# facebookresearch/SlowFast

Measured on AMD Instinct MI355X. Metric: clips/sec (fwd+bwd), SlowFast-8x8-R50 32x224^2 synthetic clips, per-GPU batch 32, higher is better.
Workload: dtype fp16; 1 GPU; SLOWFAST_8x8_R50: forward + cross_entropy loss + backward + sgd step, inputs resident in HBM, per-GPU batch 32; global_batch=32, parallelism=dp1, launch=hip-graph(fwd+bwd) + eager all-reduce/optimizer, optimizer=FlatOptimizer (fused unscale+norm+clip+update, dynamic loss scale on device)

## Files before the change

slowfast_amd/csrc/sf_api.hip:

```cpp
#include "../../include/sfamd.h"
#include "sf_bn.h"
#include "sf_common.h"
#include "sf_igemm.h"
#include "sf_igemm2.h"
#include "sf_wgrad2.h"
#include "sf_pool.h"
#include "sf_dwconv.h"
#include "sf_dwsweep.h"
#include "sf_dwtemporal.h"
#include "sf_tokens.h"
#include "sf_x3d.h"
#include "sf_stem.h"
#include "sf_attn.h"
#include "sf_roi.h"
#include "sf_optim.h"

#include <stdarg.h>
#include <stdio.h>
#include <stdlib.h>
#include <string.h>

static thread_local char g_err[512] = "";

static int fail(const char* fmt, ...) {
    va_list ap;
    va_start(ap, fmt);
    vsnprintf(g_err, sizeof(g_err), fmt, ap);
    va_end(ap);
    return -1;
}
static int check_launch(const char* what) {
    hipError_t e = hipGetLastError();
    if (e != hipSuccess) return fail("%s: launch failed: %s", what, hipGetErrorString(e));
    return 0;
}
#define REQUIRE(cond, ...) \
    do { if (!(cond)) return fail(__VA_ARGS__); } while (0)

static inline int cdiv(int64_t a, int64_t b) { return (int)((a + b - 1) / b); }
static inline int roundup(int a, int b) { return (a + b - 1) / b * b; }

static inline int test_hook(const char* name, int def) { const char* e = getenv(name); return e ? atoi(e) : def; }
#ifdef SF_DIAG
static inline int tune_knob(const char* name, int def) { const char* e = getenv(name); return e ? atoi(e) : def; }
#else
#define tune_knob(name, def) (def)
#endif

extern "C" int sf_abi_version(void) { return SF_ABI_VERSION; }
extern "C" const char* sf_backend(void) {
#ifdef SF_HOSTSIM
    return "hostsim";
#else
    return "gfx950";
#endif
}
extern "C" int sf_act_dtype(void) { return SF_ACT_DTYPE_ID; }
extern "C" const char* sf_last_error(void) { return g_err; }
#ifndef SF_BUILD_ID
#define SF_BUILD_ID "unversioned"
#endif
extern "C" const char* sf_build_id(void) {
    static const char tagged[] = "sfamd-build-id:" SF_BUILD_ID;
    return tagged + 15;
}

static int check_desc(const sf_conv_desc* d) {
    REQUIRE(d != nullptr, "conv: null descriptor");
    REQUIRE(d->N > 0 && d->Ci > 0 && d->Co > 0, "conv: empty tensor");
    REQUIRE(d->Ci % 8 == 0 && d->Co % 8 == 0, "conv: channel counts must be multiples of 8 (Ci=%d Co=%d)", d->Ci, d->Co);
    REQUIRE(d->ldx >= d->Ci && d->ldx % 8 == 0 && d->ldy >= d->Co && d->ldy % 8 == 0, "conv: bad row pitch");
    REQUIRE(d->Cw > 0 && d->Cw <= d->Ci, "conv: Cw must be in (0, Ci]");
    REQUIRE(d->Cow >= 0 && d->Cow <= d->Co, "conv: Cow must be in [0, Co]");
    REQUIRE(d->sT > 0 && d->sH > 0 && d->sW > 0 && d->dT > 0 && d->dH > 0 && d->dW > 0, "conv: stride/dilation");
    int To = (d->Ti + 2 * d->pT - d->dT * (d->kT - 1) - 1) / d->sT + 1;
    int Ho = (d->Hi + 2 * d->pH - d->dH * (d->kH - 1) - 1) / d->sH + 1;
    int Wo = (d->Wi + 2 * d->pW - d->dW * (d->kW - 1) - 1) / d->sW + 1;
    REQUIRE(d->To >= 1 && d->Ho >= 1 && d->Wo >= 1 && d->To <= To && d->Ho <= Ho && d->Wo <= Wo,
            "conv: output dims (%d,%d,%d) exceed the geometry's (%d,%d,%d)", d->To, d->Ho, d->Wo, To, Ho, Wo);
    int64_t Mo = (int64_t)d->N * d->To * d->Ho * d->Wo, Mi = (int64_t)d->N * d->Ti * d->Hi * d->Wi;
    REQUIRE(Mo < (1ll << 31) && Mi < (1ll << 31), "conv: more than 2^31 positions");
    return 0;
}

static void fill_gather_common(GatherSide& g, const sf_conv_desc* d) {
    g.kT = d->kT; g.kH = d->kH; g.kW = d->kW;
    g.strT = d->sT; g.strH = d->sH; g.strW = d->sW;
    g.padT = d->pT; g.padH = d->pH; g.padW = d->pW;
    g.dilT = d->dT; g.dilH = d->dH; g.dilW = d->dW;
    g.fdkW = make_fastdiv(d->kW);
    g.fdkH = make_fastdiv(d->kH);
    g.fdsT = make_fastdiv(d->sT);
    g.fdsH = make_fastdiv(d->sH);
    g.fdsW = make_fastdiv(d->sW);
    g.scale = nullptr; g.shift = nullptr; g.relu = 0;
    g.fdHW = make_fastdiv((uint32_t)d->Hi * (uint32_t)d->Wi);
}
static bool is_pointwise(const sf_conv_desc* d) {
    return d->kH == 1 && d->kW == 1 && d->sT == 1 && d->sH == 1 && d->sW == 1 && d->pH == 0 && d->pW == 0 &&
           d->Ho == d->Hi && d->Wo == d->Wi;
}

static GatherSide gather_fwd(const sf_conv_desc* d, const void* x, const float* sc, const float* sh, int relu) {
    GatherSide g;
    memset(&g, 0, sizeof(g));
    fill_gather_common(g, d);
    g.src = (const f16*)x; g.ld = d->ldx; g.C = d->Ci;
    g.sT = d->Ti; g.sH = d->Hi; g.sW = d->Wi;
    g.mode = 0;
    g.Ktot = d->kT * d->kH * d->kW * d->Ci;
    g.fdC = make_fastdiv(d->Ci);
    g.fdrW = make_fastdiv(d->Wo); g.fdrH = make_fastdiv(d->Ho); g.fdrT = make_fastdiv(d->To);
    g.rowT = d->To;
    g.scale = sc; g.shift = sh; g.relu = relu;
    return g;
}
static GatherSide gather_dgrad(const sf_conv_desc* d, const void* dy) {
    GatherSide g;
    memset(&g, 0, sizeof(g));
    fill_gather_common(g, d);
    g.src = (const f16*)dy; g.ld = d->ldy; g.C = d->Co;
    g.sT = d->To; g.sH = d->Ho; g.sW = d->Wo;
    g.mode = 1;
    g.Ktot = d->kT * d->kH * d->kW * d->Co;
    g.fdC = make_fastdiv(d->Co);
    g.fdrW = make_fastdiv(d->Wi); g.fdrH = make_fastdiv(d->Hi); g.fdrT = make_fastdiv(d->Ti);
    g.rowT = d->Ti;
    return g;
}

static bool igemm_glds_ok(const IgemmParams& p, bool pw) {
    static const bool off = tune_knob("SF_IGEMM_GLDS", 1) == 0;
    if (off || !pw || p.g.scale) return false;
    if (p.g.Ktot != p.g.C || p.g.Ktot % 32 != 0 || p.g.ld % 8 != 0 || p.ldw % 8 != 0) return false;
    if (p.g.padT != 0) return false;
    if (((uintptr_t)p.g.src | (uintptr_t)p.wmat) & 15) return false;
    if (p.bh > 0 && ((p.sa_b | p.sa_h | p.sw_b | p.sw_h) & 7)) return false;
    return true;
}

template <int BN, int WM, int WN>
static void launch_igemm(const IgemmParams& p, bool pw, hipStream_t s, int nbatch = 1) {
    int mt = cdiv(p.M, 128);
    dim3 grid((unsigned)(mt * p.ntiles_n), (unsigned)nbatch);
    static const bool occ4 = tune_knob("SF_IGEMM_OCC4", 1) != 0;
    if (p.f32.out) {
        if (igemm_glds_ok(p, pw)) hipLaunchKernelGGL((sf_igemm_kernel<BN, WM, WN, true, true, BN == 128, true>), grid, dim3(SF_THREADS), 0, s, p);
        else hipLaunchKernelGGL((sf_igemm_kernel<BN, WM, WN, true, false, BN == 128, true>), grid, dim3(SF_THREADS), 0, s, p);
        return;
    }
    if (igemm_glds_ok(p, pw)) {
        hipLaunchKernelGGL((sf_igemm_kernel<BN, WM, WN, true, true, BN == 128>), grid, dim3(SF_THREADS), 0, s, p);
        return;
    }
    constexpr bool kCap = BN == 128;
    const bool cap = kCap && occ4;
    if (pw) {
        if (cap) hipLaunchKernelGGL((sf_igemm_kernel<BN, WM, WN, true, false, kCap>), grid, dim3(SF_THREADS), 0, s, p);
        else hipLaunchKernelGGL((sf_igemm_kernel<BN, WM, WN, true, false, false>), grid, dim3(SF_THREADS), 0, s, p);
    } else {
        if (cap) hipLaunchKernelGGL((sf_igemm_kernel<BN, WM, WN, false, false, kCap>), grid, dim3(SF_THREADS), 0, s, p);
        else hipLaunchKernelGGL((sf_igemm_kernel<BN, WM, WN, false, false, false>), grid, dim3(SF_THREADS), 0, s, p);
    }
}

template <int BN, int BK>
static void launch_igemm2(Igemm2Params& q, hipStream_t s) {
    q.ntiles_n = cdiv(q.Nout, BN);
    const dim3 grid((unsigned)(cdiv(q.M, 256) * q.ntiles_n));
    if constexpr (BN >= 64) {
        if (q.f32.out) { hipLaunchKernelGGL((sf_igemm2_kernel<256, BN, 4, 2, BK, 3, true>), grid, dim3(512), 0, s, q); return; }
    }
    hipLaunchKernelGGL((sf_igemm2_kernel<256, BN, 4, 2, BK, 3>), grid, dim3(512), 0, s, q);
}
static void launch_igemm2_auto(Igemm2Params& q, hipStream_t s) {
    const char* e;
    const int tiles = cdiv(q.M, 256) * cdiv(q.Nout, q.Nout > 64 ? 128 : 64);
    const int force_bk = tune_knob("SF_IGEMM2_BK", 0);
    const bool bk64 = q.C % 64 == 0 && force_bk != 32 && (force_bk == 64 || tiles <= 320);
    static const bool trace = test_hook("SF_TRACE", 0) != 0;
    q.ablate = tune_knob("SF_IGEMM2_ABLATE", 0);
    if (trace) fprintf(stderr, "[sfamd] igemm2: M=%d N=%d C=%d taps=%d BK=%d omap=%d\n", q.M, q.Nout, q.C, q.ntaps, bk64 ? 64 : 32, q.omap);
    const int t128 = test_hook("SF_IGEMM2_T128", 1);
    if (t128 && q.linear && q.Nout > 64 && !q.stat_part && !q.bnb_part && (!bk64 || t128 == 2)) {
        q.ntiles_n = cdiv(q.Nout, 128);
        const dim3 grid((unsigned)(cdiv(q.M, 128) * q.ntiles_n));
        if (q.f32.out) hipLaunchKernelGGL((sf_igemm2_kernel<128, 128, 2, 2, 32, 3, true>), grid, dim3(256), 0, s, q);
        else hipLaunchKernelGGL((sf_igemm2_kernel<128, 128, 2, 2, 32, 3>), grid, dim3(256), 0, s, q);
        return;
    }
    if (q.Nout > 64) { if (bk64) launch_igemm2<128, 64>(q, s); else launch_igemm2<128, 32>(q, s); }
    else if (q.Nout > 32) { if (bk64) launch_igemm2<64, 64>(q, s); else launch_igemm2<64, 32>(q, s); }
    else launch_igemm2<32, 32>(q, s);
}
static bool igemm2_operands_ok(const IgemmParams& p, int nbatch) {
    const GatherSide& g = p.g;
    if (nbatch != 1 || g.scale) return false;
    if (p.bh > 1 || (p.bh == 1 && (p.sa_b | p.sa_h | p.sw_b | p.sw_h | p.sy_b | p.sy_h | p.sr_b | p.sr_h))) return false;
    const int taps = g.kT * g.kH * g.kW;
    if (taps > SF_I2_MAXTAPS || g.C % 32 != 0 || g.Ktot != taps * g.C) return false;
    if (g.ld % 8 != 0 || p.ldw % 8 != 0 || p.ldw < g.Ktot) return false;
    if (((uintptr_t)g.src | (uintptr_t)p.wmat) & 15) return false;
    if ((g.kT - 1) * g.dilT > 127 || (g.kH - 1) * g.dilH > 127 || (g.kW - 1) * g.dilW > 127) return false;
    return true;
}
static void igemm2_common(Igemm2Params& q, const IgemmParams& p) {
    const GatherSide& g = p.g;
    memset(&q, 0, sizeof(q));
    q.src = g.src; q.ld = g.ld; q.C = g.C;
    q.sT = g.sT; q.sH = g.sH; q.sW = g.sW;
    q.wmat = p.wmat; q.ldw = p.ldw; q.Nout = p.Nout;
    q.y = p.y; q.ldy = p.ldy; q.bias = p.bias; q.resid = p.resid; q.ldr = p.ldr; q.stat_part = p.stat_part;
    q.act_mode = p.act_mode; q.act_aux = p.act_aux; q.ld_aux = p.ld_aux; q.resid_row0 = p.resid_row0; q.alpha = p.alpha;
    q.resid_bits = p.resid_bits;
    q.bnb_y = p.bnb_y; q.bnb_ld = p.bnb_ld; q.bnb_scale = p.bnb_scale; q.bnb_shift = p.bnb_shift; q.bnb_part = p.bnb_part;
    q.bnb_bits = p.bnb_bits;
    q.f32 = p.f32;
    q.linear = p.linear;
}
static bool try_igemm2(const IgemmParams& p, hipStream_t s, int nbatch = 1) {
    const char* e;
    const bool off = test_hook("SF_IGEMM2", 1) == 0;
    const int mink = test_hook("SF_IGEMM2_MINK", 512);
    const int minrows = test_hook("SF_IGEMM2_MINROWS", 4096);
    const GatherSide& g = p.g;
    if (off || !igemm2_operands_ok(p, nbatch)) return false;
    if (g.Ktot < mink || p.Nout <= 32 || p.M < minrows) return false;
    if (g.mode == 1 && !(g.strT == 1 && g.strH == 1 && g.strW == 1)) return false;
    const int taps = g.kT * g.kH * g.kW;
    Igemm2Params q;
    igemm2_common(q, p);
    q.fdrW = g.fdrW; q.fdrH = g.fdrH; q.fdrT = g.fdrT;
    const int sgn = g.mode == 0 ? 1 : -1;
    if (g.mode == 0) {
        q.mulT = g.strT; q.mulH = g.strH; q.mulW = g.strW;
        q.offT = -g.padT; q.offH = -g.padH; q.offW = -g.padW;
    } else {
        q.mulT = q.mulH = q.mulW = 1;
        q.offT = g.padT; q.offH = g.padH; q.offW = g.padW;
    }
    q.ntaps = taps;
    int t = 0;
    for (int kt = 0; kt < g.kT; ++kt)
        for (int kh = 0; kh < g.kH; ++kh)
            for (int kw = 0; kw < g.kW; ++kw, ++t) {
                const int dt = sgn * kt * g.dilT, dh = sgn * kh * g.dilH, dw = sgn * kw * g.dilW;
                q.dt[t] = (int8_t)dt; q.dh[t] = (int8_t)dh; q.dw[t] = (int8_t)dw;
                q.taps[t].dlin = (dt * g.sH + dh) * g.sW + dw;
                q.taps[t].wcol = t * g.C;
            }
    q.M = p.M;
    launch_igemm2_auto(q, s);
    return true;
}

static bool try_igemm2_strided_dgrad(const IgemmParams& p, hipStream_t s) {
    const char* e;
    const bool off = test_hook("SF_IGEMM2", 1) == 0 || tune_knob("SF_IGEMM2_STRIDED", 1) == 0;
    const int minrows = test_hook("SF_IGEMM2_MINROWS", 4096);
    const GatherSide& g = p.g;
    if (off || g.mode != 1 || (g.strT == 1 && g.strH == 1 && g.strW == 1)) return false;
    if (!igemm2_operands_ok(p, 1) || p.Nout <= 16 || p.M < minrows || p.stat_part || p.act_mode) return false;
    const int Ti = (int)g.fdrT.d, Hi = (int)g.fdrH.d, Wi = (int)g.fdrW.d;
    const int N = p.M / (Ti * Hi * Wi);
    const int str[3] = {g.strT, g.strH, g.strW}, pad[3] = {g.padT, g.padH, g.padW}, dil[3] = {g.dilT, g.dilH, g.dilW};
    const int ker[3] = {g.kT, g.kH, g.kW}, ext[3] = {Ti, Hi, Wi};
    for (int rt = 0; rt < str[0]; ++rt)
        for (int rh = 0; rh < str[1]; ++rh)
            for (int rw = 0; rw < str[2]; ++rw) {
                const int r[3] = {rt, rh, rw};
                int q0[3], cnt[3];
                bool empty = false;
                for (int a = 0; a < 3; ++a) {
                    const int num = pad[a] - r[a];
                    q0[a] = num > 0 ? (num + str[a] - 1) / str[a] : 0;
                    const int top = ext[a] - 1 + pad[a] - r[a];
                    const int q1 = top >= 0 ? top / str[a] : -1;
                    cnt[a] = q1 - q0[a] + 1;
                    if (cnt[a] <= 0) empty = true;
                }
                if (empty) continue;
                Igemm2Params q;
                igemm2_common(q, p);
                q.fdrT = make_fastdiv(cnt[0]); q.fdrH = make_fastdiv(cnt[1]); q.fdrW = make_fastdiv(cnt[2]);
                q.mulT = q.mulH = q.mulW = 1;
                q.offT = q0[0]; q.offH = q0[1]; q.offW = q0[2];
                int nt = 0, tap = 0;
                for (int kt = 0; kt < ker[0]; ++kt)
                    for (int kh = 0; kh < ker[1]; ++kh)
                        for (int kw = 0; kw < ker[2]; ++kw, ++tap) {
                            const int k[3] = {kt, kh, kw};
                            int d[3];
                            bool ok = true;
                            for (int a = 0; a < 3; ++a) {
                                const int v = r[a] - k[a] * dil[a];
                                if (v % str[a] != 0) { ok = false; break; }
                                d[a] = v / str[a];
                            }
                            if (!ok) continue;
                            q.dt[nt] = (int8_t)d[0]; q.dh[nt] = (int8_t)d[1]; q.dw[nt] = (int8_t)d[2];
                            q.taps[nt].dlin = (d[0] * g.sH + d[1]) * g.sW + d[2];
                            q.taps[nt].wcol = tap * g.C;
                            ++nt;
                        }
                q.ntaps = nt;
                q.M = N * cnt[0] * cnt[1] * cnt[2];
                q.omap = 1;
                q.oT = Ti; q.oH = Hi; q.oW = Wi;
                q.omT = str[0]; q.omH = str[1]; q.omW = str[2];
                q.ooT = str[0] * q0[0] + r[0] - pad[0]; q.ooH = str[1] * q0[1] + r[1] - pad[1]; q.ooW = str[2] * q0[2] + r[2] - pad[2];
                launch_igemm2_auto(q, s);
            }
    return true;
}

static int run_igemm(IgemmParams& p, bool pw, hipStream_t s, int* bm_used = nullptr) {
    if (bm_used) *bm_used = 256;
    if (try_igemm2(p, s)) return check_launch("igemm2");
    if (bm_used) *bm_used = 0;
    if (try_igemm2_strided_dgrad(p, s)) return check_launch("igemm2 strided dgrad");
    if (bm_used) *bm_used = 128;
    if (p.Nout > 64) { p.ntiles_n = cdiv(p.Nout, 128); launch_igemm<128, 64, 64>(p, pw, s); }
    else if (p.Nout > 32) { p.ntiles_n = 1; launch_igemm<64, 32, 64>(p, pw, s); }
    else if (p.Nout > 16) { p.ntiles_n = 1; launch_igemm<32, 32, 32>(p, pw, s); }
    else { p.ntiles_n = 1; launch_igemm<16, 32, 16>(p, pw, s); }
    return check_launch("igemm");
}

struct StemPlan {
    bool ok, thin3, small;
    int tiles_w, tiles_h, tiles_t, ntiles, F, PR;
    int wg_blocks, tiles_per_block, Kpad, wgroups;
    size_t ws_bytes;
};
static StemPlan plan_stem(const sf_conv_desc* d) {
    StemPlan s;
    memset(&s, 0, sizeof(s));
    static const bool off = tune_knob("SF_STEM_GENERIC", 0) != 0;
    if (off) return s;
    static const bool thin3_on = tune_knob("SF_STEM_THIN3", 1) != 0;
    const bool stemlike = d->kW == 4 && d->pW == 2;
    const bool thin3 = thin3_on && d->kW == 3 && d->pW == 1 && d->sH == 1 && d->sT == 1;
    if (d->Ci != 8 || d->Cw != 8 || !(stemlike || thin3) || d->sW != 1 || d->dT != 1 || d->dH != 1 || d->dW != 1)
        return s;
    s.thin3 = thin3;
    if (d->Co > 16 || d->Co % 8 != 0 || (d->Cow && d->Cow != d->Co)) return s;
    if (d->kT * d->kH > SF_STEM_MAX_SLICES) return s;
    s.F = (SF_STEM_TT - 1) * d->sT + d->kT;
    s.PR = (SF_STEM_TH - 1) * d->sH + d->kH;
    if ((int64_t)s.F * s.PR * SF_STEM_PC > SF_STEM_CHUNKS) return s;
    s.small = (int64_t)s.F * s.PR * SF_STEM_PC <= SF_STEM_CHUNKS_SMALL;
    s.tiles_w = cdiv(d->Wo, SF_STEM_TW);
    s.tiles_h = cdiv(d->Ho, SF_STEM_TH);
    s.tiles_t = cdiv(d->To, SF_STEM_TT);
    const int64_t nt = (int64_t)d->N * s.tiles_t * s.tiles_h * s.tiles_w;
    if (nt >= (1ll << 30)) return s;
    s.ntiles = (int)nt;
    const int gmax = s.small ? 1024 : 512;
    int g = s.ntiles < gmax ? s.ntiles : gmax;
    s.tiles_per_block = cdiv(s.ntiles, g);
    s.wg_blocks = cdiv(s.ntiles, s.tiles_per_block);
    s.Kpad = roundup(d->kT * d->kH * 32, 128);
    { const int nsl = d->kT * d->kH; s.wgroups = nsl <= 4 ? 8 / nsl : 1; }
    s.ws_bytes = (size_t)s.wg_blocks * s.wgroups * 16 * s.Kpad * 4;
    s.ok = true;
    return s;
}
#define SF_STEM_SLIDE_GROUPS 4
#define SF_STEM_FWD_LAUNCH(sp, q, stream)                                                                                          \
    do {                                                                                                                          \
        static const bool rm_ = tune_knob("SF_STEM_ROWMAJOR", 1) != 0;                           \
        const dim3 g_((sp).ntiles), b_(SF_THREADS);                                                                               \
        const int sg_ = test_hook("SF_STEM_SLIDE", SF_STEM_SLIDE_GROUPS);                                                         \
        if (rm_ && sg_ > 0 && (q).sH == 2 && (q).kH == 7 && !(sp).small && (q).sT == 1 && (q).kT > 1 && (q).kT <= 5 &&            \
            (q).Co <= 8 && !(q).bnb_y) {                                                                                                         \
            StemParams qs_ = (q);                    \
            qs_.seg_groups = sg_ < (sp).tiles_t ? sg_ : (sp).tiles_t;                                                             \
            qs_.tiles_t = cdiv((sp).tiles_t, qs_.seg_groups);                                                                     \
            qs_.fd_tt = make_fastdiv(qs_.tiles_t);                                                                                \
            const dim3 gs_((unsigned)((int64_t)(q).N * qs_.tiles_t * (sp).tiles_h * (sp).tiles_w));                                \
            if (test_hook("SF_TRACE", 0)) fprintf(stderr, "[sfamd] stem_fwd_slide: %u runs of %d groups\n", gs_.x, qs_.seg_groups); \
            hipLaunchKernelGGL((sf_stem_fwd_slide_kernel<2, 7>), gs_, b_, 0, (hipStream_t)(stream), qs_);                         \
        } else if (rm_ && (q).sH == 2 && (q).kH == 7 && !(sp).small)                                                              \
            hipLaunchKernelGGL((sf_stem_fwd_kernel<SF_STEM_CHUNKS, 2, 7>), g_, b_, 0, (hipStream_t)(stream), q);                  \
        else if (rm_ && (q).sH == 1 && (q).kH == 3 && (sp).small)                                                                 \
            hipLaunchKernelGGL((sf_stem_fwd_kernel<SF_STEM_CHUNKS_SMALL, 1, 3>), g_, b_, 0, (hipStream_t)(stream), q);            \
        else if ((sp).small) hipLaunchKernelGGL((sf_stem_fwd_kernel<SF_STEM_CHUNKS_SMALL>), g_, b_, 0, (hipStream_t)(stream), q); \
        else hipLaunchKernelGGL((sf_stem_fwd_kernel<SF_STEM_CHUNKS>), g_, b_, 0, (hipStream_t)(stream), q);                       \
    } while (0)
static StemParams stem_params(const sf_conv_desc* d, const StemPlan& s, const void* x) {
    StemParams p;
    memset(&p, 0, sizeof(p));
    p.x = (const f16*)x; p.ldx = d->ldx;
    p.N = d->N; p.Ti = d->Ti; p.Hi = d->Hi; p.Wi = d->Wi;
    p.To = d->To; p.Ho = d->Ho; p.Wo = d->Wo; p.Co = d->Co;
    p.kT = d->kT; p.kH = d->kH; p.sT = d->sT; p.sH = d->sH; p.pT = d->pT; p.pH = d->pH;
    p.pW = d->pW;
    if (s.thin3) { p.wo0 = 0; p.wos = 24; p.wog = 8; p.kwc = 3; }
    else { p.wo0 = 0; p.wos = 32; p.wog = 8; p.kwc = 4; }
    p.ldy = d->ldy;
    p.tiles_w = s.tiles_w; p.tiles_h = s.tiles_h; p.tiles_t = s.tiles_t; p.ntiles = s.ntiles;
    p.fd_tw = make_fastdiv(s.tiles_w); p.fd_th = make_fastdiv(s.tiles_h); p.fd_tt = make_fastdiv(s.tiles_t);
    p.F = s.F; p.PR = s.PR;
    p.fd_pc = make_fastdiv(SF_STEM_PC); p.fd_prpc = make_fastdiv(s.PR * SF_STEM_PC);
    p.Kpad = s.Kpad; p.tiles_per_block = s.tiles_per_block; p.wgroups = s.wgroups;
    return p;
}

extern "C" int sf_conv_weight_ld(const sf_conv_desc* d, int32_t* ldf, int32_t* ldd) {
    REQUIRE(d && ldf && ldd, "sf_conv_weight_ld: null argument");
    int taps = d->kT * d->kH * d->kW;
    *ldf = roundup(taps * d->Ci, 32);
    *ldd = roundup(taps * d->Co, 32);
    return 0;
}

static PrepParams prep_params(const sf_conv_desc* d, const float* w, void* wf, void* wd) {
    PrepParams p;
    memset(&p, 0, sizeof(p));
    p.w = w; p.Co = d->Co; p.Cow = d->Cow ? d->Cow : d->Co; p.Cw = d->Cw; p.Cp = d->Ci; p.taps = d->kT * d->kH * d->kW;
    int32_t ldf, ldd;
    sf_conv_weight_ld(d, &ldf, &ldd);
    p.wf = (f16*)wf; p.ldf = ldf; p.wd = (f16*)wd; p.ldd = ldd;
    return p;
}

extern "C" int sf_prep_weights(const sf_conv_desc* d, const float* w, void* wf, void* wd, sf_stream_t stream) {
    if (check_desc(d)) return -1;
    REQUIRE(w && wf, "sf_prep_weights: null pointer");
    const PrepParams p = prep_params(d, w, wf, wd);
    int64_t total = (int64_t)p.Co * p.ldf + (wd ? (int64_t)p.Cp * p.ldd : 0);
    int blocks = (int)((total + SF_THREADS - 1) / SF_THREADS);
    if (blocks > 4096) blocks = 4096;
    hipLaunchKernelGGL(sf_prep_weights_kernel, dim3(blocks), dim3(SF_THREADS), 0, (hipStream_t)stream, p);
    return check_launch("prep_weights");
}

static_assert(sizeof(sf_prep_item) == sizeof(PrepParams), "sf_prep_item must mirror PrepParams");
extern "C" int sf_prep_item_fill(const sf_conv_desc* d, const float* w, void* wf, void* wd, sf_prep_item* item) {
    if (check_desc(d)) return -1;
    REQUIRE(w && wf && item, "sf_prep_item_fill: null pointer");
    PrepParams p = prep_params(d, w, wf, wd);
    p.pad = sf_prep_tile_co(p.taps);
    memcpy(item, &p, sizeof(p));
    return 0;
}

extern "C" int64_t sf_prep_item_blocks(const sf_prep_item* item) {
    REQUIRE(item && item->Co > 0 && item->ldf > 0 && item->taps > 0, "sf_prep_item_blocks: bad item");
    REQUIRE(item->pad == sf_prep_tile_co(item->taps), "sf_prep_item_blocks: item was not written by sf_prep_item_fill");
    if (item->pad > 0) return (int64_t)cdiv(item->Co, item->pad) * cdiv(item->Cp, SF_PREP_TILE_CI);
    const int64_t n = (int64_t)item->Co * item->ldf + (item->wd ? (int64_t)item->Cp * item->ldd : 0);
    return cdiv(n, SF_PREP_BLOCK_ELEMS);
}

extern "C" int sf_prep_weights_batch(const sf_prep_item* items, const int32_t* blk_item, const int32_t* blk_off,
                                     int32_t nblocks, sf_stream_t stream) {
    REQUIRE(items && blk_item && blk_off && nblocks > 0, "sf_prep_weights_batch: bad arguments");
    hipLaunchKernelGGL(sf_prep_weights_batch_kernel, dim3(nblocks), dim3(SF_THREADS), 0, (hipStream_t)stream,
                       (const PrepParams*)items, blk_item, blk_off);
    return check_launch("prep_weights_batch");
}

extern "C" int sf_conv_fwd_mtiles(const sf_conv_desc* d) {
    if (!d) return fail("sf_conv_fwd_mtiles: null descriptor");
    return cdiv((int64_t)d->N * d->To * d->Ho * d->Wo, 128);
}

extern "C" int sf_conv_fwd(const sf_conv_desc* d, const void* x, const void* wf, const float* in_scale,
                           const float* in_shift, int in_relu, const float* bias, void* y, float* stat_part,
                           sf_stream_t stream) {
    if (check_desc(d)) return -1;
    REQUIRE(x && wf && y, "sf_conv_fwd: null pointer");
    REQUIRE((in_scale == nullptr) == (in_shift == nullptr), "sf_conv_fwd: in_scale/in_shift must come together");
    REQUIRE(!in_scale || d->Ci <= 512, "sf_conv_fwd: fused input BatchNorm supports Ci <= 512 (got %d)", d->Ci);
    if (!in_scale && !bias) {
        const StemPlan sp = plan_stem(d);
        if (sp.ok && (!stat_part || sp.ntiles <= sf_conv_fwd_mtiles(d))) {
            StemParams q = stem_params(d, sp, x);
            int32_t ldf0, ldd0;
            sf_conv_weight_ld(d, &ldf0, &ldd0);
            q.wmat = (const f16*)wf; q.ldw = ldf0; q.y = (f16*)y;
            q.stat_part = stat_part; q.stat_rows = sf_conv_fwd_mtiles(d);
            const bool trace = test_hook("SF_TRACE", 0) != 0;
            if (trace) fprintf(stderr, "[sfamd] stem_fwd: %d tiles, patch %dx%dx%d chunks\n", sp.ntiles, sp.F, sp.PR, SF_STEM_PC);
            SF_STEM_FWD_LAUNCH(sp, q, stream);
            return check_launch("stem_fwd");
        }
    }
    IgemmParams p;
    memset(&p, 0, sizeof(p));
    p.g = gather_fwd(d, x, in_scale, in_shift, in_relu);
    p.M = d->N * d->To * d->Ho * d->Wo;
    int32_t ldf, ldd;
    sf_conv_weight_ld(d, &ldf, &ldd);
    p.wmat = (const f16*)wf; p.ldw = ldf; p.Nout = d->Co;
    p.ksteps = cdiv(p.g.Ktot, 32);
    p.y = (f16*)y; p.ldy = d->ldy;
    p.bias = bias; p.resid = nullptr; p.ldr = 0;
    p.stat_part = stat_part;
    return run_igemm(p, is_pointwise(d), (hipStream_t)stream);
}

extern "C" int sf_conv_fwd_fused(const sf_conv_desc* d, const void* x, const void* wf, const float* bias,
                                 const void* resid, int32_t ldr, int out_relu, void* y, sf_stream_t stream) {
    if (check_desc(d)) return -1;
    REQUIRE(x && wf && y, "sf_conv_fwd_fused: null pointer");
    REQUIRE(!resid || (ldr >= d->Co && ldr % 8 == 0), "sf_conv_fwd_fused: bad residual pitch");
    if (!resid) {
        const StemPlan sp = plan_stem(d);
        if (sp.ok) {
            StemParams q = stem_params(d, sp, x);
            int32_t ldf0, ldd0;
            sf_conv_weight_ld(d, &ldf0, &ldd0);
            q.wmat = (const f16*)wf; q.ldw = ldf0; q.y = (f16*)y;
            q.bias = bias; q.out_relu = out_relu;
            SF_STEM_FWD_LAUNCH(sp, q, stream);
            return check_launch("stem_fwd_fused");
        }
    }
    IgemmParams p;
    memset(&p, 0, sizeof(p));
    p.g = gather_fwd(d, x, nullptr, nullptr, 0);
    p.M = d->N * d->To * d->Ho * d->Wo;
    int32_t ldf, ldd;
    sf_conv_weight_ld(d, &ldf, &ldd);
    p.wmat = (const f16*)wf; p.ldw = ldf; p.Nout = d->Co;
    p.ksteps = cdiv(p.g.Ktot, 32);
    p.y = (f16*)y; p.ldy = d->ldy;
    p.bias = bias; p.resid = (const f16*)resid; p.ldr = ldr;
    p.act_mode = out_relu ? 3 : 0;
    return run_igemm(p, is_pointwise(d), (hipStream_t)stream);
}

struct BnFuse {
    const float* scale; const float* shift; const void* bits;
    const void* y0; int32_t ld0; float* part0;
};
static int conv_dgrad_impl(const sf_conv_desc* d, const void* dy, const void* wd, const void* resid, int32_t ldr,
                           const void* resid_bits, void* dx, const BnFuse* bn, int32_t* bn_rows, sf_stream_t stream) {
    if (check_desc(d)) return -1;
    REQUIRE(dy && wd && dx, "sf_conv_dgrad: null pointer");
    REQUIRE(!resid || (ldr >= d->Ci && ldr % 8 == 0), "sf_conv_dgrad: bad residual pitch");
    IgemmParams p;
    memset(&p, 0, sizeof(p));
    p.g = gather_dgrad(d, dy);
    p.M = d->N * d->Ti * d->Hi * d->Wi;
    int32_t ldf, ldd;
    sf_conv_weight_ld(d, &ldf, &ldd);
    p.wmat = (const f16*)wd; p.ldw = ldd; p.Nout = d->Ci;
    p.ksteps = cdiv(p.g.Ktot, 32);
    p.y = (f16*)dx; p.ldy = d->ldx;
    p.resid = (const f16*)resid; p.ldr = ldr;
    REQUIRE(!resid_bits || resid, "sf_conv_dgrad: resid_bits without a residual");
    p.resid_bits = (const uint8_t*)resid_bits;
    const bool fuse = bn && d->sT == 1 && d->sH == 1 && d->sW == 1;
    if (!resid && d->Co == 8 && d->To == d->Ti && d->Ho == d->Hi && d->Wo == d->Wi) {
        sf_conv_desc dd = *d;
        dd.Ci = d->Co; dd.Cw = d->Co; dd.Co = d->Ci; dd.Cow = 0;
        dd.pT = d->kT - 1 - d->pT; dd.pH = d->kH - 1 - d->pH; dd.pW = d->kW - 1 - d->pW;
        dd.ldx = d->ldy; dd.ldy = d->ldx;
        const StemPlan sp = plan_stem(&dd);
        if (sp.ok && sp.thin3 && (!fuse || sp.ntiles <= cdiv(p.M, 128))) {
            StemParams q = stem_params(&dd, sp, dy);
            const int S = d->kT * d->kH;
            q.wmat = (const f16*)wd; q.ldw = ldd; q.y = (f16*)dx;
            q.wo0 = ((S - 1) * 3 + 2) * 8; q.wos = -24; q.wog = -8; q.kwc = 3;
            if (fuse) {
                q.bnb_y = (const f16*)bn->y0; q.bnb_ld = bn->ld0; q.bnb_scale = bn->scale; q.bnb_shift = bn->shift;
                q.bnb_bits = (const uint8_t*)bn->bits;
                q.stat_part = bn->part0; q.stat_rows = 0;
            }
            SF_STEM_FWD_LAUNCH(sp, q, stream);
            if (bn_rows) *bn_rows = fuse ? sp.ntiles : 0;
            return check_launch("stem_dgrad");
        }
    }
    if (fuse) {
        p.bnb_y = (const f16*)bn->y0; p.bnb_ld = bn->ld0; p.bnb_part = bn->part0;
        p.bnb_scale = bn->scale; p.bnb_shift = bn->shift; p.bnb_bits = (const uint8_t*)bn->bits;
    }
    int bm = 0;
    const int rc = run_igemm(p, is_pointwise(d), (hipStream_t)stream, &bm);
    if (bn_rows) *bn_rows = (fuse && bm > 0) ? cdiv(p.M, bm) : 0;
    return rc;
}

extern "C" int sf_conv_dgrad(const sf_conv_desc* d, const void* dy, const void* wd, const void* resid, int32_t ldr,
                             const void* resid_bits, void* dx, sf_stream_t stream) {
    return conv_dgrad_impl(d, dy, wd, resid, ldr, resid_bits, dx, nullptr, nullptr, stream);
}

extern "C" int sf_conv_dgrad_bn(const sf_conv_desc* d, const void* dy, const void* wd, const void* resid, int32_t ldr,
                                const void* resid_bits, void* dx, const float* mask_scale, const float* mask_shift,
                                const void* mask_bits, const void* bn_y, int32_t bn_ldy, float* bn_part, int32_t bn_part_rows,
                                int32_t* bn_rows, sf_stream_t stream) {
    REQUIRE(d && bn_y && bn_part && bn_rows, "sf_conv_dgrad_bn: null pointer");
    REQUIRE(mask_bits || (mask_scale && mask_shift), "sf_conv_dgrad_bn: a mask source is needed (mask_bits, or mask_scale + mask_shift)");
    REQUIRE(bn_ldy >= d->Ci && bn_ldy % 8 == 0 && ((uintptr_t)bn_y & 15) == 0, "sf_conv_dgrad_bn: bad bn_y pitch / alignment");
    REQUIRE((int64_t)bn_part_rows * 128 >= (int64_t)d->N * d->Ti * d->Hi * d->Wi,
            "sf_conv_dgrad_bn: the partial table needs ceil(positions / 128) rows of [2][Ci] floats");
    const BnFuse bn = {mask_scale, mask_shift, mask_bits, bn_y, bn_ldy, bn_part};
    return conv_dgrad_impl(d, dy, wd, resid, ldr, resid_bits, dx, &bn, bn_rows, stream);
}

template <int BMW, int WM, int WN, int KS>
static void launch_wgrad(WgradParams& p, dim3 grid3, hipStream_t s) {
    p.tiles_k = grid3.x; p.tiles_c = grid3.y;
    const dim3 grid(grid3.x * grid3.y * grid3.z);
    hipLaunchKernelGGL((sf_wgrad_kernel<BMW, WM, WN, KS>), grid, dim3(SF_THREADS), 0, s, p);
}

struct WgradPlan {
    int BMW, KS, tiles_k, tiles_c, Co_pad, Kpad, nchunks, chunks_per_split, splits;
    size_t ws_bytes;
};
static WgradPlan plan_wgrad(const sf_conv_desc* d) {
    WgradPlan w;
    const int taps = d->kT * d->kH * d->kW;
    const int Ktot = taps * d->Ci;
    const int64_t M = (int64_t)d->N * d->To * d->Ho * d->Wo;
    w.BMW = d->Co >= 128 ? 128 : d->Co >= 64 ? 64 : d->Co >= 32 ? 32 : 16;
    w.KS = w.BMW <= 32 ? 4 : 1;
    w.tiles_k = cdiv(Ktot, 128);
    w.tiles_c = cdiv(d->Co, w.BMW);
    w.Kpad = w.tiles_k * 128;
    w.Co_pad = w.tiles_c * w.BMW;
    w.nchunks = cdiv(M, 32);
    const int64_t slab = (int64_t)w.Co_pad * w.Kpad * 4;
    static const int target = tune_knob("SF_WGRAD_BLOCKS", 1024);
    int splits = cdiv(target, (int64_t)w.tiles_k * w.tiles_c);
    const int64_t cap = (256ll << 20) / slab;
    if (splits > cap) splits = (int)(cap < 1 ? 1 : cap);
    const int nstages = cdiv(w.nchunks, w.KS);
    if (splits > nstages) splits = nstages;
    if (splits < 1) splits = 1;
    w.chunks_per_split = cdiv(nstages, splits) * w.KS;
    w.splits = cdiv(w.nchunks, w.chunks_per_split);
    w.ws_bytes = (size_t)slab * w.splits;
    return w;
}

struct Wgrad2Plan {
    bool ok, thin, dual;
    int BMW, BKW, tiles_k, tiles_c, Co_pad, Kpad, rows_per_split, splits;
    int slabs;
    size_t tab_bytes, ws_bytes;
};
static Wgrad2Plan plan_wgrad2(const sf_conv_desc* d) {
    Wgrad2Plan w;
    memset(&w, 0, sizeof(w));
    const char* e;
    if (test_hook("SF_WGRAD2", 1) == 0) return w;
    const int mink = test_hook("SF_WGRAD2_MINK", 192);
    const int minrows = test_hook("SF_WGRAD2_MINROWS", 4096);
    const int taps = d->kT * d->kH * d->kW;
    const int target = test_hook("SF_WGRAD2_BLOCKS", 512);
    (void)taps;
    const int Ktot = taps * d->Ci;
    const int64_t M = (int64_t)d->N * d->To * d->Ho * d->Wo;
    if (taps > SF_I2_MAXTAPS || M < minrows) return w;
    if ((d->kT - 1) * d->dT > 127 || (d->kH - 1) * d->dH > 127 || (d->kW - 1) * d->dW > 127) return w;
    if (plan_stem(d).ok) return w;
    if (d->Co <= 32) {
        if (test_hook("SF_WGRAD2T", 1) == 0) return w;
        const int minrows_t = test_hook("SF_WGRAD2T_MINROWS", 16384);
        if (M < minrows_t) return w;
        w.thin = true;
        w.BMW = d->Co <= 16 ? 16 : 32;
        w.BKW = Ktot <= 32 ? 32 : 128;
        w.tiles_k = cdiv(Ktot, w.BKW);
        w.tiles_c = 1;
        w.Kpad = w.tiles_k * w.BKW;
        w.Co_pad = w.BMW;
        const int target_t = test_hook("SF_WGRAD2T_BLOCKS", w.BKW == 128 ? 512 : w.BMW == 32 ? 768 : 1024);
        int splits = target_t / w.tiles_k;
        if (splits < 1) splits = 1;
        w.rows_per_split = roundup(cdiv(M, splits), 128);
        w.splits = cdiv(M, w.rows_per_split);
        w.tab_bytes = ((size_t)M * 8 + 255) / 256 * 256 + 1280;
        w.ws_bytes = w.tab_bytes + (size_t)w.Co_pad * w.Kpad * 4 * w.splits;
        w.slabs = w.splits;
        w.ok = true;
        return w;
    }
    if (Ktot < mink) return w;
    w.BMW = d->Co > 64 ? 128 : 64;
    w.tiles_k = cdiv(Ktot, 256);
    w.tiles_c = cdiv(d->Co, w.BMW);
    w.Kpad = w.tiles_k * 256;
    w.Co_pad = w.tiles_c * w.BMW;
    int splits = target / (w.tiles_k * w.tiles_c);
    const int64_t slab = (int64_t)w.Co_pad * w.Kpad * 4;
    const int64_t cap = (256ll << 20) / slab;
    if (splits > cap) splits = (int)(cap < 1 ? 1 : cap);
    if (splits < 1) splits = 1;
    w.dual = false;
    if (splits >= 2 && test_hook("SF_WGRAD2_DUAL", 1) != 0) {
        const int tiles = w.tiles_k * w.tiles_c;
        const int pairs = (target / 2) / tiles;
        const int64_t steps = cdiv(cdiv(M, splits), 32);
        if (pairs >= 1 && 2 * pairs * 10 >= (2 * pairs < splits ? splits : 2 * pairs) * 9 && steps <= test_hook("SF_WGRAD2_DUAL_STEPS", 80)) {
            w.dual = true;
            if (2 * pairs < splits) splits = 2 * pairs;
        }
    }
    w.rows_per_split = roundup(cdiv(M, splits), 32);
    w.splits = cdiv(M, w.rows_per_split);
    if (w.splits < 2) w.dual = false;
    w.slabs = w.dual ? cdiv(w.splits, 2) : w.splits;
    w.tab_bytes = ((size_t)M * 8 + 255) / 256 * 256 + 1280;
    w.ws_bytes = w.tab_bytes + (size_t)slab * w.splits;
    w.ok = true;
    return w;
}

static void launch_rowtab(const sf_conv_desc* d, void* tab, hipStream_t s) {
    RowtabParams t;
    memset(&t, 0, sizeof(t));
    t.tab = (i32x2*)tab;
    t.M = d->N * d->To * d->Ho * d->Wo;
    t.fdW = make_fastdiv(d->Wo); t.fdH = make_fastdiv(d->Ho); t.fdT = make_fastdiv(d->To);
    t.sT = d->Ti; t.sH = d->Hi; t.sW = d->Wi;
    t.strT = d->sT; t.strH = d->sH; t.strW = d->sW; t.padT = d->pT; t.padH = d->pH; t.padW = d->pW;
    t.ntaps = d->kT * d->kH * d->kW;
    int ti = 0;
    for (int kt = 0; kt < d->kT; ++kt)
        for (int kh = 0; kh < d->kH; ++kh)
            for (int kw = 0; kw < d->kW; ++kw, ++ti) {
                t.dt[ti] = (int8_t)(kt * d->dT); t.dh[ti] = (int8_t)(kh * d->dH); t.dw[ti] = (int8_t)(kw * d->dW);
            }
    hipLaunchKernelGGL(sf_wgrad2_rowtab_kernel, dim3(cdiv(t.M, SF_THREADS)), dim3(SF_THREADS), 0, s, t);
}

extern "C" int64_t sf_conv_wgrad_rowtab_bytes(const sf_conv_desc* d) {
    if (check_desc(d)) return -1;
    const Wgrad2Plan w2 = plan_wgrad2(d);
    return w2.ok ? (int64_t)w2.tab_bytes : 0;
}

extern "C" int sf_conv_wgrad_rowtab(const sf_conv_desc* d, void* tab, sf_stream_t stream) {
    if (check_desc(d)) return -1;
    REQUIRE(tab && (uintptr_t)tab % 16 == 0, "sf_conv_wgrad_rowtab: tab must be a 16-byte aligned device pointer");
    REQUIRE(plan_wgrad2(d).ok, "sf_conv_wgrad_rowtab: this geometry does not take the row-table kernel (sf_conv_wgrad_rowtab_bytes == 0)");
    launch_rowtab(d, tab, (hipStream_t)stream);
    return check_launch("wgrad_rowtab");
}

extern "C" int64_t sf_conv_wgrad_workspace(const sf_conv_desc* d) {
    if (check_desc(d)) return -1;
    int64_t generic = (int64_t)plan_wgrad(d).ws_bytes;
    const Wgrad2Plan w2 = plan_wgrad2(d);
    if (w2.ok && (int64_t)w2.ws_bytes > generic) generic = (int64_t)w2.ws_bytes;
    const StemPlan sp = plan_stem(d);
    return sp.ok && (int64_t)sp.ws_bytes > generic ? (int64_t)sp.ws_bytes : generic;
}

extern "C" int sf_conv_wgrad(const sf_conv_desc* d, const void* x, const float* in_scale, const float* in_shift,
                             int in_relu, const void* dy, float* dw, float out_scale, int zero_first,
                             void* workspace, int64_t workspace_bytes, const void* rowtab, sf_stream_t stream) {
    if (check_desc(d)) return -1;
    REQUIRE(x && dy && dw && workspace, "sf_conv_wgrad: null pointer");
    REQUIRE((in_scale == nullptr) == (in_shift == nullptr), "sf_conv_wgrad: in_scale/in_shift must come together");
    REQUIRE(!in_scale || d->Ci <= 512, "sf_conv_wgrad: fused input BatchNorm supports Ci <= 512 (got %d)", d->Ci);
    hipStream_t s = (hipStream_t)stream;
    int splits, Co_pad, Kpad;
    GatherSide gk = gather_fwd(d, x, in_scale, in_shift, in_relu);
    const StemPlan sp = plan_stem(d);
    const Wgrad2Plan w2 = in_scale ? Wgrad2Plan{} : plan_wgrad2(d);
    float* slabs = (float*)workspace;
    if (w2.ok) {
        REQUIRE(workspace_bytes >= (int64_t)w2.ws_bytes, "sf_conv_wgrad: workspace too small (%lld < %lld bytes)",
                (long long)workspace_bytes, (long long)w2.ws_bytes);
        REQUIRE(((uintptr_t)x | (uintptr_t)dy | (uintptr_t)workspace) % 16 == 0, "sf_conv_wgrad: operands must be 16-byte aligned");
        Wgrad2Params q;
        memset(&q, 0, sizeof(q));
        int ti = 0;
        for (int kt = 0; kt < d->kT; ++kt)
            for (int kh = 0; kh < d->kH; ++kh)
                for (int kw = 0; kw < d->kW; ++kw, ++ti) q.dlin[ti] = (kt * d->dT * d->Hi + kh * d->dH) * d->Wi + kw * d->dW;
        if (!rowtab) launch_rowtab(d, workspace, s);
        else REQUIRE((uintptr_t)rowtab % 16 == 0, "sf_conv_wgrad: rowtab must be 16-byte aligned");
        q.x = (const f16*)x; q.ldx = d->ldx; q.C = d->Ci;
        q.dy = (const f16*)dy; q.ldy = d->ldy; q.Co = d->Co;
        q.M = d->N * d->To * d->Ho * d->Wo; q.Ktot = gk.Ktot;
        q.rowtab = (const i32x2*)(rowtab ? rowtab : workspace);
        slabs = (float*)((char*)workspace + w2.tab_bytes);
        q.ws = slabs; q.Co_pad = w2.Co_pad; q.Kpad = w2.Kpad;
        q.tiles_k = w2.tiles_k; q.tiles_c = w2.tiles_c; q.rows_per_split = w2.rows_per_split;
        q.stage_stride = (w2.thin && tune_knob("SF_WGRAD2T_RR", 1) != 0) ? w2.splits : 0;
        const dim3 grid((unsigned)(w2.tiles_k * w2.tiles_c * w2.slabs));
        static const bool trace = test_hook("SF_TRACE", 0) != 0;
        if (trace) fprintf(stderr, "[sfamd] wgrad2: M=%d Co=%d K=%d tiles %dx%d splits %d%s\n", q.M, q.Co, q.Ktot, w2.tiles_c, w2.tiles_k, w2.splits,
                           w2.dual ? " (two per workgroup)" : "");
        if (w2.thin) {
            if (w2.BMW == 16 && w2.BKW == 128) hipLaunchKernelGGL((sf_wgrad2t_kernel<16, 128, 2>), grid, dim3(256), 0, s, q);
            else if (w2.BMW == 32 && w2.BKW == 128) hipLaunchKernelGGL((sf_wgrad2t_kernel<32, 128, 2>), grid, dim3(256), 0, s, q);
            else if (w2.BMW == 16) hipLaunchKernelGGL((sf_wgrad2t_kernel<16, 32, 3>), grid, dim3(256), 0, s, q);
            else hipLaunchKernelGGL((sf_wgrad2t_kernel<32, 32, 3>), grid, dim3(256), 0, s, q);
        } else if (w2.dual) {
            if (w2.BMW == 128) hipLaunchKernelGGL((sf_wgrad2_kernel<128, true>), grid, dim3(1024), 0, s, q);
            else hipLaunchKernelGGL((sf_wgrad2_kernel<64, true>), grid, dim3(1024), 0, s, q);
        } else {
            if (w2.BMW == 128) hipLaunchKernelGGL((sf_wgrad2_kernel<128>), grid, dim3(512), 0, s, q);
            else hipLaunchKernelGGL((sf_wgrad2_kernel<64>), grid, dim3(512), 0, s, q);
        }
        splits = w2.slabs; Co_pad = w2.Co_pad; Kpad = w2.Kpad;
    } else if (sp.ok && !in_scale) {
        REQUIRE(workspace_bytes >= (int64_t)sp.ws_bytes, "sf_conv_wgrad: workspace too small (%lld < %lld bytes)",
                (long long)workspace_bytes, (long long)sp.ws_bytes);
        StemParams q = stem_params(d, sp, x);
        q.dy = (const f16*)dy; q.ws = (float*)workspace;
        const bool trace = test_hook("SF_TRACE", 0) != 0;
        if (trace) fprintf(stderr, "[sfamd] stem_wgrad: %d workgroups x %d tiles\n", sp.wg_blocks, sp.tiles_per_block);
        static const bool stem_plain = tune_knob("SF_STEM_XCD", 1) == 0;
        q.plain_order = stem_plain ? 1 : 0;
        if (d->Co <= 8 && sp.small) hipLaunchKernelGGL((sf_stem_wgrad_kernel<8, SF_STEM_CHUNKS_SMALL>), dim3(sp.wg_blocks), dim3(SF_STEM_WG_THREADS), 0, s, q);
        else if (d->Co <= 8) hipLaunchKernelGGL((sf_stem_wgrad_kernel<8, SF_STEM_CHUNKS>), dim3(sp.wg_blocks), dim3(SF_STEM_WG_THREADS), 0, s, q);
        else if (sp.small) hipLaunchKernelGGL((sf_stem_wgrad_kernel<16, SF_STEM_CHUNKS_SMALL>), dim3(sp.wg_blocks), dim3(SF_STEM_WG_THREADS), 0, s, q);
        else hipLaunchKernelGGL((sf_stem_wgrad_kernel<16, SF_STEM_CHUNKS>), dim3(sp.wg_blocks), dim3(SF_STEM_WG_THREADS), 0, s, q);
        splits = sp.wg_blocks * sp.wgroups; Co_pad = 16; Kpad = sp.Kpad;
    } else {
        const WgradPlan w = plan_wgrad(d);
        REQUIRE(workspace_bytes >= (int64_t)w.ws_bytes, "sf_conv_wgrad: workspace too small (%lld < %lld bytes)",
                (long long)workspace_bytes, (long long)w.ws_bytes);
        REQUIRE(w.splits <= 65535, "sf_conv_wgrad: too many splits");
        WgradParams p;
        memset(&p, 0, sizeof(p));
        p.g = gk;
        p.dy = (const f16*)dy; p.ldy = d->ldy; p.Co = d->Co;
        p.M = d->N * d->To * d->Ho * d->Wo;
        p.ws = (float*)workspace; p.Co_pad = w.Co_pad; p.Kpad = w.Kpad;
        p.nchunks = w.nchunks; p.chunks_per_split = w.chunks_per_split;
        dim3 grid(w.tiles_k, w.tiles_c, w.splits);
        switch (w.BMW) {
            case 128: launch_wgrad<128, 64, 64, 1>(p, grid, s); break;
            case 64: launch_wgrad<64, 32, 64, 1>(p, grid, s); break;
            case 32: launch_wgrad<32, 32, 32, 4>(p, grid, s); break;
            default: launch_wgrad<16, 16, 32, 4>(p, grid, s); break;
        }
        splits = w.splits; Co_pad = w.Co_pad; Kpad = w.Kpad;
    }
    if (check_launch("wgrad")) return -1;
    WgradReduceParams r;
    r.ws = slabs; r.splits = splits; r.Co = d->Cow ? d->Cow : d->Co; r.Co_pad = Co_pad; r.Kpad = Kpad;
    r.Ktot = gk.Ktot; r.fdC = gk.fdC; r.dw = dw; r.Cw = d->Cw; r.taps = d->kT * d->kH * d->kW;
    r.slice4 = 0;
    if (sp.ok && sp.thin3 && !in_scale && !w2.ok) { r.slice4 = 1; r.Ktot = d->kT * d->kH * 32; }
    r.out_scale = out_scale; r.accumulate = zero_first ? 0 : 1;
    int64_t total = (int64_t)r.Co * Kpad / 4;
    int lanes = 1;
    while (lanes < 32 && lanes * 4 <= splits) lanes *= 2;
    r.lanes = lanes;
    const int per_block = SF_THREADS / lanes;
    hipLaunchKernelGGL(sf_wgrad_reduce_kernel, dim3(cdiv(total, per_block)), dim3(SF_THREADS), 0, s, r);
    return check_launch("wgrad_reduce");
}

static RowTile make_rowtile(int64_t M, int C, int max_blocks, dim3& grid) {
    RowTile rt;
    rt.M = (int)M; rt.C = C;
    const int G = C / 8;
    const int TG = G < SF_THREADS ? G : SF_THREADS;
    const int rpi = SF_THREADS / TG;
    int passes = cdiv(M, (int64_t)rpi * max_blocks);
    if (passes < 1) passes = 1;
    rt.rows_per_block = rpi * passes;
    grid = dim3(cdiv(M, rt.rows_per_block), cdiv(G, SF_THREADS));
    return rt;
}
static int check_rows(const char* who, int64_t M, int C) {
    REQUIRE(M > 0 && M < (1ll << 31), "%s: bad row count", who);
    REQUIRE(C > 0 && C % 8 == 0, "%s: C must be a positive multiple of 8 (got %d)", who, C);
    return 0;
}

static const int kFoldAbove = tune_knob("SF_FOLD_ABOVE", 2048);
static int fold_partials(float* part, int& nblk, int C, hipStream_t s) {
// ... 1706 lines not shown
```

Measured before the change: 870.3 clips/s.

## Add LDS-patch direct conv kernel for 64-channel 3x3 convs in fwd and dgrad

After: 878.6 clips/s, median of 6. Within noise of the previous version (+1.0%).

```diff
diff --git a/slowfast_amd/csrc/sf_api.hip b/slowfast_amd/csrc/sf_api.hip
--- a/slowfast_amd/csrc/sf_api.hip
+++ b/slowfast_amd/csrc/sf_api.hip
@@ -11,6 +11,7 @@
 #include "sf_tokens.h"
 #include "sf_x3d.h"
 #include "sf_stem.h"
+#include "sf_patch64.h"
 #include "sf_attn.h"
 #include "sf_roi.h"
 #include "sf_optim.h"
@@ -407,6 +408,39 @@
     return p;
 }
 
+struct Patch64Plan { bool ok; int tiles_w, tiles_h, ntiles, tiles_per_block, blocks; };
+static Patch64Plan plan_patch64(const sf_conv_desc* d) {
+    Patch64Plan s;
+    memset(&s, 0, sizeof(s));
+    if (test_hook("SF_PATCH64", 1) == 0) return s;
+    if (d->Ci != 64 || d->Co != 64 || d->Cw != 64 || (d->Cow && d->Cow != 64)) return s;
+    if (d->kT != 1 || d->kH != 3 || d->kW != 3 || d->pT != 0 || d->pH != 1 || d->pW != 1) return s;
+    if (d->sT != 1 || d->sH != 1 || d->sW != 1 || d->dT != 1 || d->dH != 1 || d->dW != 1) return s;
+    if (d->To != d->Ti || d->Ho != d->Hi || d->Wo != d->Wi) return s;
+    if (d->ldx % 8 != 0 || d->ldy % 8 != 0) return s;
+    const int64_t M = (int64_t)d->N * d->Ti * d->Hi * d->Wi;
+    if (M < test_hook("SF_PATCH64_MINROWS", 4096)) return s;
+    s.tiles_w = cdiv(d->Wi, SF_P64_TW);
+    s.tiles_h = cdiv(d->Hi, SF_P64_TH);
+    const int64_t nt = (int64_t)d->N * d->Ti * s.tiles_h * s.tiles_w;
+    if (nt >= (1ll << 30)) return s;
+    s.ntiles = (int)nt;
+    int64_t g = cdiv(M, 128);
+    if (g > SF_P64_MAXBLOCKS) g = SF_P64_MAXBLOCKS;
+    s.tiles_per_block = cdiv(s.ntiles, g);
+    s.blocks = cdiv(s.ntiles, s.tiles_per_block);
+    s.ok = true;
+    return s;
+}
+static Patch64Params patch64_params(const sf_conv_desc* d, const Patch64Plan& s) {
+    Patch64Params q;
+    memset(&q, 0, sizeof(q));
+    q.NT = d->N * d->Ti; q.H = d->Hi; q.W = d->Wi;
+    q.tiles_w = s.tiles_w; q.tiles_h = s.tiles_h; q.ntiles = s.ntiles; q.tiles_per_block = s.tiles_per_block;
+    q.fd_tw = make_fastdiv(s.tiles_w); q.fd_th = make_fastdiv(s.tiles_h);
+    return q;
+}
+
 extern "C" int sf_conv_weight_ld(const sf_conv_desc* d, int32_t* ldf, int32_t* ldd) {
     REQUIRE(d && ldf && ldd, "sf_conv_weight_ld: null argument");
     int taps = d->kT * d->kH * d->kW;
@@ -486,6 +520,19 @@
             if (trace) fprintf(stderr, "[sfamd] stem_fwd: %d tiles, patch %dx%dx%d chunks\n", sp.ntiles, sp.F, sp.PR, SF_STEM_PC);
             SF_STEM_FWD_LAUNCH(sp, q, stream);
             return check_launch("stem_fwd");
+        }
+    }
+    if (!in_scale && !bias && (((uintptr_t)x | (uintptr_t)wf | (uintptr_t)y) & 15) == 0) {
+        const Patch64Plan pp = plan_patch64(d);
+        if (pp.ok) {
+            Patch64Params q = patch64_params(d, pp);
+            int32_t ldf0, ldd0;
+            sf_conv_weight_ld(d, &ldf0, &ldd0);
+            q.src = (const f16*)x; q.ld = d->ldx; q.wmat = (const f16*)wf; q.ldw = ldf0; q.y = (f16*)y; q.ldy = d->ldy;
+            q.stat_part = stat_part; q.stat_rows = sf_conv_fwd_mtiles(d);
+            if (test_hook("SF_TRACE", 0)) fprintf(stderr, "[sfamd] patch64_fwd: %d tiles on %d workgroups\n", pp.ntiles, pp.blocks);
+            hipLaunchKernelGGL((sf_patch64_kernel<false>), dim3(pp.blocks), dim3(256), 0, (hipStream_t)stream, q);
+            return check_launch("patch64_fwd");
         }
     }
     IgemmParams p;
@@ -574,6 +621,21 @@
             SF_STEM_FWD_LAUNCH(sp, q, stream);
             if (bn_rows) *bn_rows = fuse ? sp.ntiles : 0;
             return check_launch("stem_dgrad");
+        }
+    }
+    if (!resid && (((uintptr_t)dy | (uintptr_t)wd | (uintptr_t)dx) & 15) == 0) {
+        const Patch64Plan pp = plan_patch64(d);
+        if (pp.ok) {
+            Patch64Params q = patch64_params(d, pp);
+            q.src = (const f16*)dy; q.ld = d->ldy; q.wmat = (const f16*)wd; q.ldw = ldd; q.y = (f16*)dx; q.ldy = d->ldx;
+            if (fuse) {
+                q.bnb_y = (const f16*)bn->y0; q.bnb_ld = bn->ld0; q.bnb_scale = bn->scale; q.bnb_shift = bn->shift;
+                q.bnb_bits = (const uint8_t*)bn->bits; q.bnb_part = bn->part0;
+            }
+            if (test_hook("SF_TRACE", 0)) fprintf(stderr, "[sfamd] patch64_dgrad: %d tiles on %d workgroups\n", pp.ntiles, pp.blocks);
+            hipLaunchKernelGGL((sf_patch64_kernel<true>), dim3(pp.blocks), dim3(256), 0, (hipStream_t)stream, q);
+            if (bn_rows) *bn_rows = fuse ? pp.blocks : 0;
+            return check_launch("patch64_dgrad");
         }
     }
     if (fuse) {
diff --git a/slowfast_amd/csrc/sf_patch64.h b/slowfast_amd/csrc/sf_patch64.h
--- /dev/null
+++ b/slowfast_amd/csrc/sf_patch64.h
@@ -0,0 +1,176 @@
+#pragma once
+#include "sf_common.h"
+#include "sf_igemm.h"
+
+#define SF_P64_TH 8
+#define SF_P64_TW 16
+#define SF_P64_PR (SF_P64_TH + 2)
+#define SF_P64_PW 24
+#define SF_P64_PATCH (SF_P64_PR * SF_P64_PW * 64)
+#define SF_P64_COPIES (SF_P64_PR * SF_P64_PW / 8)
+#define SF_P64_MAXBLOCKS 512
+
+struct Patch64Params {
+    const f16* src; int ld;
+    int NT, H, W;
+    const f16* wmat; int ldw;
+    f16* y; int ldy;
+    float* stat_part; int stat_rows;
+    const f16* bnb_y; int bnb_ld; const float* bnb_scale; const float* bnb_shift; const uint8_t* bnb_bits;
+    float* bnb_part;
+    int tiles_w, tiles_h, ntiles, tiles_per_block;
+    FastDiv fd_tw, fd_th;
+};
+
+template <bool FLIP>
+__global__ __launch_bounds__(256, 2) void sf_patch64_kernel(Patch64Params p) {
+    constexpr int STG_LD = 64 + 8;
+    static_assert(128 * STG_LD <= SF_P64_PATCH, "the staged tile fits a patch buffer");
+    static_assert(4 * 8 * 24 * 4 <= SF_P64_PATCH * 2, "the reduction scratch fits a patch buffer");
+    __shared__ __attribute__((aligned(16))) f16 lds[2 * SF_P64_PATCH];
+    const int tid = threadIdx.x, lane = tid & 63, wave = __builtin_amdgcn_readfirstlane(tid >> 6);
+    const int pl = lane & 15, g4 = lane >> 4;
+    const int bid = (int)xcd_remap(blockIdx.x, gridDim.x);
+    const int tile_begin = bid * p.tiles_per_block;
+    const int tile_end = tile_begin + p.tiles_per_block < p.ntiles ? tile_begin + p.tiles_per_block : p.ntiles;
+    const f16* const zline = reinterpret_cast<const f16*>(sf_zero_line);
+    const int64_t plane_stride = (int64_t)p.H * p.W * p.ld;
+
+    f16x8 wreg[18];
+    {
+        const f16* wrow = p.wmat + (int64_t)(wave * 16 + pl) * p.ldw + g4 * 8;
+#pragma unroll
+        for (int ks = 0; ks < 18; ++ks) wreg[ks] = ld16(wrow + ks * 32);
+    }
+
+    const int cslot = (lane & 7) ^ (lane >> 3);
+    auto issue = [&](int tile, int buf) {
+        const uint32_t a = fd_div((uint32_t)tile, p.fd_tw);
+        const int w0 = (int)((uint32_t)tile - a * (uint32_t)p.tiles_w) * SF_P64_TW;
+        const uint32_t pln = fd_div(a, p.fd_th);
+        const int h0 = (int)(a - pln * (uint32_t)p.tiles_h) * SF_P64_TH;
+        const f16* base = p.src + (int64_t)pln * plane_stride + cslot * 8;
+        f16* dst = lds + buf * SF_P64_PATCH;
+#pragma unroll
+        for (int u = 0; u < (SF_P64_COPIES + 3) / 4; ++u) {
+            const int j = wave + 4 * u;
+            if (j < SF_P64_COPIES) {
+                const int pr = j / 3, pc = (j - pr * 3) * 8 + (lane >> 3);
+                const int h = h0 - 1 + pr, w = w0 - 1 + pc;
+                const bool ok = pc < SF_P64_TW + 2 && (unsigned)h < (unsigned)p.H && (unsigned)w < (unsigned)p.W;
+                const f16* g = ok ? base + (int64_t)(h * p.W + w) * p.ld : zline;
+                SF_GLOBAL_LOAD_LDS16_ASM(g, dst + j * 512);
+            }
+        }
+    };
+
+    int aoff[3][2];
+#pragma unroll
+    for (int dw = 0; dw < 3; ++dw)
+#pragma unroll
+        for (int kk = 0; kk < 2; ++kk) aoff[dw][kk] = (pl + dw) * 64 + (((kk * 4 + g4) ^ ((pl + dw) & 7)) << 3);
+
+    float ssum = 0.f, qsum = 0.f;
+    const int ecg = tid & 7;
+    float bsg[8], bsgy[8], bsc[8], bsh[8];
+#pragma unroll
+    for (int e = 0; e < 8; ++e) { bsg[e] = 0.f; bsgy[e] = 0.f; bsc[e] = 1.f; bsh[e] = 0.f; }
+    const bool bnb = p.bnb_part != nullptr;
+    if (bnb && !p.bnb_bits) { load8f(p.bnb_scale + ecg * 8, bsc); load8f(p.bnb_shift + ecg * 8, bsh); }
+
+    if (tile_begin < tile_end) issue(tile_begin, 0);
+    for (int tile = tile_begin; tile < tile_end; ++tile) {
+        const int buf = (tile - tile_begin) & 1;
+        SF_WAIT_VMEM();
+        SF_BARRIER_KEEP_VMEM();
+        if (tile + 1 < tile_end) issue(tile + 1, buf ^ 1);
+        const f16* patch = lds + buf * SF_P64_PATCH;
+
+        f32x4 acc[SF_P64_TH];
+#pragma unroll
+        for (int i = 0; i < SF_P64_TH; ++i) acc[i] = (f32x4){0.f, 0.f, 0.f, 0.f};
+        auto frag = [&](int s, f16x8 (&a)[SF_P64_TH]) {
+            const int tap = s >> 1, kk = s & 1, kh = tap / 3, kw = tap - kh * 3;
+            const int dh = FLIP ? 2 - kh : kh, dw = FLIP ? 2 - kw : kw;
+#pragma unroll
+            for (int i = 0; i < SF_P64_TH; ++i) a[i] = ld16(patch + (i + dh) * (SF_P64_PW * 64) + aoff[dw][kk]);
+        };
+        f16x8 a0[SF_P64_TH], a1[SF_P64_TH];
+        frag(0, a0);
+#pragma unroll
+        for (int s = 0; s < 18; s += 2) {
+            frag(s + 1, a1);
+            __builtin_amdgcn_sched_barrier(0);
+#pragma unroll
+            for (int i = 0; i < SF_P64_TH; ++i) acc[i] = SF_MFMA16(a0[i], wreg[s], acc[i]);
+            __builtin_amdgcn_sched_barrier(0);
+            if (s + 2 < 18) frag(s + 2, a0);
+            __builtin_amdgcn_sched_barrier(0);
+#pragma unroll
+            for (int i = 0; i < SF_P64_TH; ++i) acc[i] = SF_MFMA16(a1[i], wreg[s + 1], acc[i]);
+            __builtin_amdgcn_sched_barrier(0);
+        }
+
+        const uint32_t ta = fd_div((uint32_t)tile, p.fd_tw);
+        const int w0 = (int)((uint32_t)tile - ta * (uint32_t)p.tiles_w) * SF_P64_TW;
+        const uint32_t pln = fd_div(ta, p.fd_th);
+        const int h0 = (int)(ta - pln * (uint32_t)p.tiles_h) * SF_P64_TH;
+        if (p.stat_part) {
+#pragma unroll
+            for (int i = 0; i < SF_P64_TH; ++i)
+#pragma unroll
+                for (int r = 0; r < 4; ++r) {
+                    const bool ok = h0 + i < p.H && w0 + 4 * g4 + r < p.W;
+                    const float v = ok ? acc[i][r] : 0.f;
+                    ssum += v;
+                    qsum += v * v;
+                }
+        }
+        SF_BARRIER_KEEP_VMEM();
+        f16* stg = lds + buf * SF_P64_PATCH;
+#pragma unroll
+        for (int i = 0; i < SF_P64_TH; ++i)
+#pragma unroll
+            for (int r = 0; r < 4; ++r) stg[(i * 16 + 4 * g4 + r) * STG_LD + wave * 16 + pl] = (f16)acc[i][r];
+        SF_BARRIER_KEEP_VMEM();
+        const int64_t row0 = (int64_t)pln * p.H * p.W;
+        EpiLoads L[4];
+        bool ok[4];
+        int64_t mo[4];
+#pragma unroll
+        for (int u = 0; u < 4; ++u) {
+            const int row = (tid >> 3) + 32 * u;
+            const int h = h0 + (row >> 4), w = w0 + (row & 15);
+            ok[u] = h < p.H && w < p.W;
+            mo[u] = ok[u] ? row0 + h * p.W + w : 0;
+            L[u].bbits = 0u;
+            if (ok[u] && bnb) {
+                L[u].y = ld16(p.bnb_y + mo[u] * p.bnb_ld + ecg * 8);
+                if (p.bnb_bits) L[u].bbits = p.bnb_bits[mo[u] * 8 + ecg];
+            }
+        }
+#pragma unroll
+        for (int u = 0; u < 4; ++u) {
+            if (!ok[u]) continue;
+            const int row = (tid >> 3) + 32 * u;
+            const f16x8 v = ld16(stg + row * STG_LD + ecg * 8);
+            st16(p.y + mo[u] * p.ldy + ecg * 8, v);
+            if (bnb) bnb_accumulate(v, L[u].y, bsc, bsh, bsg, bsgy, p.bnb_bits != nullptr, L[u].bbits);
+        }
+    }
+
+    if (p.stat_part) {
+        ssum = wave_sum_over_row_groups(ssum);
+        qsum = wave_sum_over_row_groups(qsum);
+        if (lane < 16) {
+            p.stat_part[((int64_t)bid * 2 + 0) * 64 + wave * 16 + lane] = ssum;
+            p.stat_part[((int64_t)bid * 2 + 1) * 64 + wave * 16 + lane] = qsum;
+        }
+        if (tid < 128)
+            for (int64_t row = (int64_t)bid + gridDim.x; row < p.stat_rows; row += gridDim.x) p.stat_part[row * 128 + tid] = 0.f;
+    }
+    if (bnb) {
+        SF_WAIT_VMEM();
+        bnb_reduce_store<4, 8>(bsg, bsgy, reinterpret_cast<float*>(lds), p.bnb_part + (int64_t)bid * 2 * 64, 0, 64);
+    }
+}
```
